# pvjosue/CWFA

Measured on AMD Instinct MI355X. Metric: volumes/sec inverse-pass @512×512×96 fp32; NLL match vs ref (1/2/4/8 GPU), higher is better.
Workload: dtype f32 (storage, accumulation, wavelets, couplings); convolution products on the bf16 matrix cores from an exact three-way bf16 split of both fp32 operands, six products per fp32 product: fp32-equivalent; plain-fp32-MFMA figure: fp32_mfma; 1 GPU; 512x512x96 volume, 4-scale CWFA (CAT blocks, 64 ch) + LRNN inverse, z=0, batch 1/GPU, random-init weights (BASELINE.json configs[2]); precision=split, parallelism=replicated x1 (independent volumes per GPU, no collective)

## Files before the change

cwfa_amd/_lib.py:

```python
import ctypes as C
import os

_HERE = os.path.dirname(os.path.abspath(__file__))
LIB_PATH = os.path.join(_HERE, "libcwfa_hip.so")

CLAMP = {"NONE": 0, "ATAN": 1, "TANH": 2, "SIGMOID": 3}
ACT = {None: 0, "none": 0, "elu": 1, "prelu": 2, "gelu": 3, "relu": 4}
CHAIN_MAX = 8

c_f32p = C.c_void_p
c_i64p = C.c_void_p
c_f64p = C.c_void_p


class AffineStage(C.Structure):
    _fields_ = [("s_raw", c_f32p), ("t", c_f32p), ("s_bs", C.c_int64), ("t_bs", C.c_int64), ("clamp_kind", C.c_int),
                ("clamp", C.c_float), ("pre_scale", C.c_float), ("t_neg_div_sqrt2", C.c_int), ("perm", c_i64p),
                ("perm_axis", C.c_int), ("gin", C.c_int)]


class Chain(C.Structure):
    _fields_ = [("n_stages", C.c_int), ("stage", AffineStage * CHAIN_MAX), ("src_c", C.c_void_p), ("src_h", C.c_void_p)]


# ... 37 lines not shown
    "cwfa_haar2d_inv_f32": (i, [p, p, i, i, i, i, i, f, p]),
    "cwfa_haar3d_fwd_f32": (i, [p, p, i, i, i, i, i, f, i64, p]),
    "cwfa_haar3d_inv_f32": (i, [p, p, i, i, i, i, i, f, i64, p]),
    "cwfa_gather_f32": (i, [p, p, p, i, i, i, i, i, i64, i64, p]),
    "cwfa_affine_f32": (i, [p, p, C.POINTER(AffineStage), i, i, i, i, i, i64, i64, p, p, p]),
    "cwfa_channel_affine_f32": (i, [p, p, p, p, i, p, p, i, i, i64, i64, i64, p]),
    "cwfa_chain_inv_f32": (i, [p, p, p, C.POINTER(Chain), i, i, i, i, i64, i64, i64, p, p]),
    "cwfa_chain_fwd_f32": (i, [p, p, p, C.POINTER(Chain), p, i, i, i, i, i64, i64, i64, p, p, p]),
    "cwfa_conv2d_packed_floats": (i64, [i, i, i]),
    "cwfa_conv2d_pack_f32": (i, [p, p, i, i, i, i, p]),
    "cwfa_conv2d_f32": (i, [p, p, p, i, i, i, i, i, i, i64, i64, C.POINTER(ConvOpts), p]),
    "cwfa_subnet_pack1x1_f32": (i, [p, p, p]),
    "cwfa_subnet_layer_tape_f32": (i, [p, p, p, p, p, p, p, i, i, i, i64, i64, i64, p]),
    "cwfa_subnet_layer_f32": (i, [p, p, p, p, p, p, i, i, i, i64, i64, p]),
    "cwfa_conv3d_1k1_f32": (i, [p, p, p, p, p, p, p, i, i, i, i, i, p]),
    "cwfa_conv3d_1k1_split_f32": (i, [p, p, p, p, p, p, p, i, i, i, i, i, p]),
    "cwfa_channel_stats_f32": (i, [p, p, i, i, i64, i64, p]),
    "cwfa_bn_fold_f32": (i, [p, d, p, p, p, p, f, p, i, p, p, i, p]),
    "cwfa_maxpool_f32": (i, [p, p, p, p, p, i, i, i, i, i, i, p]),
    "cwfa_sample_stats_f32": (i, [p, p, i, i64, p]),
    "cwfa_layernorm_apply_f32": (i, [p, p, p, p, f, p, i, i64, p]),
    "cwfa_attention_combine_f32": (i, [p, p, p, p, p, p, p, p, i, i, i64, p]),
    "cwfa_scale_channels_f32": (i, [p, p, p, i, i, i64, p]),
    "cwfa_axpby_f32": (i, [p, p, f, f, p, i64, p]),
    "cwfa_bn_running_update_f32": (i, [p, C.c_double, f, p, p, p, i, p]),
    "cwfa_bn_finish_f32": (i, [p, d, p, p, p, f, i, p, p, f, p, p, f, f, i, p, p, i, i, p]),
    "cwfa_chain_bwd_f32": (i, [p, p, C.POINTER(Chain), C.POINTER(ChainGrads), p, p, i, i, i, i, i64, i64, i64, f, f, i, p, p]),
    "cwfa_affine_bwd_f32": (i, [p, p, C.POINTER(AffineStage), i, i, i, i, i, i64, i64, p, p, p, p, p]),
    "cwfa_chain_inv_bwd_f32": (i, [p, p, C.POINTER(Chain), C.POINTER(ChainGrads), i, i, i, i, i64, i64, f, i, i, p, p, p, p]),
    "cwfa_conv2d_wgrad_workspace_bytes": (i64, [i, i, i, i, i, i]),
    "cwfa_conv2d_wgrad_f32": (i, [p, p, p, p, p, i, i, i, i, i, i, i64, i64, f, p]),
    "cwfa_elu_bwd_f32": (i, [p, p, p, p, i, i64, i64, i64, i64, i64, p]),
    "cwfa_conv3d_hidden_fwd_f32": (i, [p, p, p, p, i, i, i, i, i, p]),
    "cwfa_conv3d_hidden_bwd_f32": (i, [p, p, p, p, p, p, i, i, i, i, i, p]),
    "cwfa_conv3d_input_bwd_f32": (i, [p, p, p, i, i, i, i, i, p]),
    "cwfa_conv3d_wgrad_workspace_bytes": (i64, [i, i, i, i]),
    "cwfa_conv3d_wgrad_f32": (i, [p, p, p, p, p, i, i, i, i, i, i, i, f, p]),
    "cwfa_prelu_bwd_f32": (i, [p, p, p, p, p, i, i64, i64, i64, i64, p]),
    "cwfa_plane_affine_f32": (i, [p, p, p, i, p, p, i, i, i64, i64, i64, i64, p]),
    "cwfa_bn_bwd_stats_f32": (i, [p, p, p, p, i, i, i64, i64, i64, p]),
    "cwfa_bn_act_bwd_f32": (i, [p, p, p, i, p, p, p, p, p, i, i, i64, i64, i64, i64, p]),
    "cwfa_maxpool2_bwd_f32": (i, [p, p, p, p, i, i, i, i, p]),
    "cwfa_gelu_f32": (i, [p, p, p, i64, i, p]),
    "cwfa_layernorm_bwd_f32": (i, [p, p, p, p, p, p, p, p, p, i, i64, p]),
    "cwfa_attention_bwd_f32": (i, [p, p, p, p, p, p, p, p, p, i, i, i64, p]),
    "cwfa_split_workspace_bytes": (i64, [i, i, i64]),
    "cwfa_split_input_f32": (i, [p, p, i, i, i64, i64, p, p, i64, p, i64, p]),
    "cwfa_conv_split_packed_bytes": (i64, [i, i, i]),
    "cwfa_conv_split_pack_f32": (i, [p, p, i, i, i, i, p]),
    "cwfa_conv_split_f32": (i, [p, p, p, i, i, i, i, i, i, i64, C.POINTER(ConvOpts), p]),
    "cwfa_conv3x3_split_packed_bytes": (i64, [i, i]),
    "cwfa_conv3x3_split_pack_f32": (i, [p, p, i, i, p]),
    "cwfa_conv3x3_split_f32": (i, [p, p, p, i, i, i, i, i, i64, i64, C.POINTER(ConvOpts), p]),
    "cwfa_conv7x7_split_packed_bytes": (i64, [i, i]),
    "cwfa_conv7x7_split_pack_f32": (i, [p, p, i, i, p]),
    "cwfa_conv7x7_split_f32": (i, [p, p, p, i, i, i, i, i, i64, i64, C.POINTER(ConvOpts), p]),
    "cwfa_couple_rows": (i, [i, p]),
    "cwfa_conv3x3_split_couple_f32": (i, [p, p, p, i, i, i, i, i64, C.POINTER(Couple), p]),
    "cwfa_subnet_layer_split_packed_bytes": (i64, []),
    "cwfa_subnet_layer_split_pack_f32": (i, [p, p, p, p]),
    "cwfa_subnet_layer_split_f32": (i, [p, p, p, p, p, i, i, i, i64, i64, i, p]),
    "cwfa_subnet_layer_split_tape_f32": (i, [p, p, p, p, p, p, i, i, i, i64, i64, i64, p]),
    "cwfa_subnet_layer_first_packed_bytes": (i64, []),
    "cwfa_subnet_layer_first_pack_f32": (i, [p, p, p, i, p, p]),
    "cwfa_subnet_layer_first_f32": (i, [p, p, p, p, p, p, i, i, i, i, i64, i64, i64, i, p]),
    "cwfa_extract_views_f32": (i, [p, p, p, i, i, i, i, i, i, f, f, i64, p]),
    "cwfa_eval_splits": (i64, [i, i64]),
    "cwfa_volume_extrema_f32": (i, [p, p, p, p, i, i64, i64, i64, C.POINTER(EvalAffine), p]),
    "cwfa_volume_metrics_f32": (i, [p, p, p, p, i, i64, i64, i64, C.POINTER(EvalAffine), f, f, f, p]),
    "cwfa_mip3_f32": (i, [p, p, p, p, p, p, i, i, i, i, i64, i64, i, C.POINTER(EvalAffine), C.POINTER(EvalPost), p]),
    "cwfa_projection_compose_f32": (i, [p, p, p, p, p, i, i, i, i, i, i, i, p]),
    "cwfa_roi_means_f32": (i, [p, p, p, i, i, i, i, i, i64, p]),
    "cwfa_select_positive_f32": (i, [p, i, i64, i64, i64, p, p, p, p]),
}
del i, i64, f, d, p

_lib = None


class CwfaHipError(RuntimeError):
    pass


def lib():
    global _lib
    if _lib is None:
        if not os.path.exists(LIB_PATH):
            raise CwfaHipError(
                f"{LIB_PATH} not found: build the HIP extension first (python -m cwfa_amd.build, or "
                f"__graft_entry__.build()).  cwfa_amd has no CPU / PyTorch fallback.")
        import torch
        h = C.CDLL(LIB_PATH)
        for name, (res, args) in SIGNATURES.items():
            fn = getattr(h, name)
            fn.restype = res
            fn.argtypes = args
        if h.cwfa_version() < 100:
            raise CwfaHipError("libcwfa_hip.so is older than this Python layer")
        _lib = h
    return _lib


def check(rc, what=""):
    if rc != 0:
        msg = lib().cwfa_last_error()
        raise CwfaHipError(f"{what or 'libcwfa_hip'} failed (code {rc}): {msg.decode() if msg else ''}")
# ... 1 lines not shown
```

cwfa_amd/build.py:

```python
import os
import subprocess
import sys
from concurrent.futures import ThreadPoolExecutor

HERE = os.path.dirname(os.path.abspath(__file__))
CSRC = os.path.join(HERE, "csrc")
INCLUDE = os.path.join(os.path.dirname(HERE), "include")
LIB = os.path.join(HERE, "libcwfa_hip.so")
SOURCES = ["elementwise.hip", "conv2d.hip", "conv_wino.hip", "conv_wino2d.hip", "conv_split_layer.hip", "conv_split3x3.hip", "conv3d.hip", "conv3d_split.hip", "lrnn_ops.hip", "conv_bwd.hip", "eval_ops.hip"]
HIPCC = os.environ.get("HIPCC", "/opt/rocm/bin/hipcc")
FLAGS = ["--offload-arch=gfx950", "-O3", "-fPIC", "-std=c++17", "-ffp-contract=off", "-I", INCLUDE, "-I", CSRC,
         "-Wall", "-Wno-unused-function"]


EXTRA = {"conv3d_split.hip": ["-fno-slp-vectorize"]}


def _newer(src, dst):
    return not os.path.exists(dst) or os.path.getmtime(src) > os.path.getmtime(dst)


def build_all(force=False, verbose=False):
    deps = [os.path.join(CSRC, "common.h"), os.path.join(CSRC, "conv_internal.h"), os.path.join(INCLUDE, "cwfa_hip.h"),
            os.path.abspath(__file__)]
    objs, jobs = [], []
    for s in SOURCES:
        src, obj = os.path.join(CSRC, s), os.path.join(CSRC, s.replace(".hip", ".o"))
        objs.append(obj)
        if force or _newer(src, obj) or any(_newer(d, obj) for d in deps):
            jobs.append([HIPCC, *FLAGS, *EXTRA.get(s, []), "-c", src, "-o", obj])

    def run(cmd):
        if verbose:
            print(" ".join(cmd), flush=True)
        r = subprocess.run(cmd, capture_output=True, text=True)
        if r.returncode != 0:
            raise RuntimeError(f"hipcc failed: {' '.join(cmd)}\n{r.stdout}\n{r.stderr}")
        return r.stderr

    with ThreadPoolExecutor(max_workers=4) as ex:
        for warn in ex.map(run, jobs):
            if verbose and warn.strip():
                print(warn, file=sys.stderr)
    if jobs or force or not os.path.exists(LIB) or any(_newer(o, LIB) for o in objs):
        run([HIPCC, "--offload-arch=gfx950", "-shared", "-fPIC", "-o", LIB, *objs])
    return LIB


if __name__ == "__main__":
    print(build_all(force="--force" in sys.argv, verbose=True))
```

cwfa_amd/csrc/conv2d.hip:

```cpp
#include "conv_internal.h"

#include <string.h>
#include <type_traits>

namespace {

template <int KS_, int CK_, int MT_, int NT_, int WM_, int WN_, int XV_ = 1>
struct Cfg {
    static constexpr int KS = KS_, CK = CK_, MT = MT_, NT = NT_, WM = WM_, WN = WN_;
    static constexpr int XV = XV_;
    static_assert(XV_ == 1 || (XV_ == 4 && KS_ == 1), "vector staging needs halo-free tiles");
    static constexpr int PAD = KS / 2;
    static constexpr int NTHREADS = 64 * WM * WN;
    static constexpr int CT = 32 * MT * WM;
    static constexpr int TR = NT * WN;
    static constexpr int TC = 32;
    static constexpr int XR = TR + KS - 1;
    static constexpr int XC = TC + KS - 1;
    static constexpr int XS = CK * XR * XC;
    static constexpr int XS_PAD = (XS + 3) & ~3;
    static constexpr int WS = KS * KS * CK * CT;
    static constexpr int XPT = (XS / XV + NTHREADS - 1) / NTHREADS;
    static constexpr int WPT = (WS / 4 + NTHREADS - 1) / NTHREADS;
    static constexpr int BUF = XS_PAD + WS;
// ... 503 lines not shown
    p.tiles_y = (p.H + C::TR - 1) / C::TR;
    p.nchunks = (p.Cin + C::CK - 1) / C::CK;
    const int ctiles = (p.Cout + C::CT - 1) / C::CT;
    CWFA_REQUIRE((int64_t)p.tiles_x * p.tiles_y < (1ll << 31) && ctiles <= 65535 && p.B <= 65535, CWFA_E_SHAPE,
                 "cwfa_conv2d_f32: grid too large");
    CWFA_REQUIRE((int64_t)(p.Cin + C::CK) * p.H * p.W * 4 < (1ll << 31), CWFA_E_SHAPE,
                 "cwfa_conv2d_f32: one sample's input must stay below 2 GiB (32-bit buffer offsets)");
    grid = dim3((unsigned)(p.tiles_x * p.tiles_y), ctiles, p.B);
    return CWFA_OK;
}

template <class C, int EPI, bool PRO>
int launch_epi(ConvParams p, hipStream_t stream) {
    dim3 grid;
    int rc = prepare<C>(p, grid);
    if (rc) return rc;
    constexpr int LDS = EPI == EPI_GENERIC && C::LDS_BYTES < C::NTHREADS * 64 ? C::NTHREADS * 64 : C::LDS_BYTES;
    rc = cwfa_max_lds<&conv2d_mfma_kernel<C, EPI, PRO>>(LDS, "cwfa_conv2d_f32");
    if (rc) return rc;
    hipLaunchKernelGGL((conv2d_mfma_kernel<C, EPI, PRO>), grid, dim3(C::NTHREADS), LDS, stream, p);
    CWFA_LAUNCH_CHECK("cwfa_conv2d_f32");
    return CWFA_OK;
}

template <class C, unsigned ALLOWED, bool PRO>
int launch_sel(const ConvParams& p, int epi, hipStream_t st) {
    if (!(ALLOWED & (1u << epi)) && epi != EPI_NONE_BLK8) epi = EPI_GENERIC;
    switch (epi) {
        case EPI_NONE: if constexpr (ALLOWED & (1u << EPI_NONE)) return launch_epi<C, EPI_NONE, PRO>(p, st); break;
        case EPI_ELU: if constexpr (ALLOWED & (1u << EPI_ELU)) return launch_epi<C, EPI_ELU, PRO>(p, st); break;
        case EPI_RES_ELU: if constexpr (ALLOWED & (1u << EPI_RES_ELU)) return launch_epi<C, EPI_RES_ELU, PRO>(p, st); break;
        case EPI_PRELU: if constexpr (ALLOWED & (1u << EPI_PRELU)) return launch_epi<C, EPI_PRELU, PRO>(p, st); break;
        case EPI_RES_PRELU: if constexpr (ALLOWED & (1u << EPI_RES_PRELU)) return launch_epi<C, EPI_RES_PRELU, PRO>(p, st); break;
        case EPI_GELU_RES: if constexpr (ALLOWED & (1u << EPI_GELU_RES)) return launch_epi<C, EPI_GELU_RES, PRO>(p, st); break;
        case EPI_UP: if constexpr (ALLOWED & (1u << EPI_UP)) return launch_epi<C, EPI_UP, PRO>(p, st); break;
        case EPI_NONE_BLK8:
            if constexpr (ALLOWED & (1u << EPI_NONE_BLK8)) return launch_epi<C, EPI_NONE_BLK8, PRO>(p, st);
            cwfa_set_error("cwfa_conv2d_f32: out_blocked8 is built for the 1x1 kernels with more than 32 output channels");
            return CWFA_E_SHAPE;
        default: break;
    }
    return launch_epi<C, EPI_GENERIC, PRO>(p, st);
}

template <class C, unsigned ALLOWED, unsigned ALLOWED_PRO>
int launch(const ConvParams& p, int epi, hipStream_t st) {
    if (p.o.in_scale || p.o.in_add) return launch_sel<C, ALLOWED_PRO, true>(p, epi, st);
    return launch_sel<C, ALLOWED, false>(p, epi, st);
}

}
int g_cwfa_split_xcd_map = 1;
int g_cwfa_split_rows16 = 1;
extern int g_cwfa_mip3_ablate;
namespace {

int fill_params(ConvParams& p, const char* name, const float* x, const float* w_packed, float* y, int B, int Cin, int H,
                int W, int Cout, int64_t x_bs, int64_t y_bs, const cwfa_conv_opts* opts) {
    CWFA_REQUIRE(B >= 0 && Cin > 0 && Cout > 0 && H >= 0 && W >= 0, CWFA_E_INVAL, "%s: bad size", name);
    if (B == 0 || H == 0 || W == 0) return 1;
    CWFA_REQUIRE(x && w_packed && y, CWFA_E_INVAL, "%s: null pointer", name);
    CWFA_REQUIRE((int64_t)Cin * H * W < (1ll << 30) && (int64_t)Cout * H * W * (p.o.upshuffle2 ? 1 : 1) < (1ll << 30), CWFA_E_SHAPE, "%s: C*H*W exceeds the 32-bit byte offsets of a tile (2^30 elements per image)", name);
    CWFA_REQUIRE(cwfa_aligned16(w_packed), CWFA_E_ALIGN, "%s: packed weights must be 16-byte aligned", name);
    p.x = x; p.wp = w_packed; p.y = y;
    p.B = B; p.Cin = Cin; p.H = H; p.W = W; p.Cout = Cout;
    p.x_bs = x_bs; p.y_bs = y_bs;
    p.products = g_cwfa_operand == CwfaOperand::split3 ? 6 : 1;
    if (opts) p.o = *opts;
    CWFA_REQUIRE(!(p.o.in_scale && !p.o.in_shift), CWFA_E_INVAL, "%s: in_scale without in_shift", name);
    CWFA_REQUIRE(p.o.act >= 0 && p.o.act <= CWFA_ACT_RELU && p.o.act2 >= 0 && p.o.act2 <= CWFA_ACT_RELU, CWFA_E_INVAL,
                 "%s: bad activation", name);
    CWFA_REQUIRE(!((p.o.act == CWFA_ACT_PRELU || p.o.act2 == CWFA_ACT_PRELU) && !p.o.prelu_alpha), CWFA_E_INVAL,
                 "%s: PReLU without prelu_alpha", name);
    return CWFA_OK;
}

typedef Cfg<1, 16, 2, 4, 4, 2> CS;
constexpr int CS_XB = 3 * 2 * 8 * 32 * 16, CS_WB = 3 * 2 * 256 * 16, CS_BUFB = CS_XB + CS_WB;

__device__ __forceinline__ void split3(float v, unsigned short (&o)[3]) {
    const __bf16 a1 = (__bf16)v;
    const float r1 = v - (float)a1;
    const __bf16 a2 = (__bf16)r1;
    const float r2 = r1 - (float)a2;
    const __bf16 a3 = (__bf16)r2;
    o[0] = __builtin_bit_cast(unsigned short, a1);
    o[1] = __builtin_bit_cast(unsigned short, a2);
    o[2] = __builtin_bit_cast(unsigned short, a3);
}

__device__ __forceinline__ unsigned short f16_bits(float v) { return __builtin_bit_cast(unsigned short, (_Float16)v); }

template <bool F16 = false>
__global__ __launch_bounds__(256) void split_input_kernel(const float* __restrict__ x, uint4* __restrict__ ws, int Cin, int CG2,
                                                          int64_t HW, int64_t x_bs, const float* __restrict__ sc,
                                                          const float* __restrict__ sh, int64_t aff_bs,
                                                          const float* __restrict__ add, int64_t add_bs) {
    const int64_t px = (int64_t)blockIdx.x * 256 + threadIdx.x;
    if (px >= HW) return;
    const int cg = blockIdx.y, b = blockIdx.z;
    unsigned short pc[3][8];
#pragma unroll
    for (int j = 0; j < 8; ++j) {
        const int c = cg * 8 + j;
        float v = 0.f;
        if (c < Cin) {
// ... 240 lines not shown
    if (rc) return rc < 0 ? rc : CWFA_OK;
    ConvParams& p = sp.c;
    CWFA_REQUIRE(!p.o.in_scale && !p.o.in_add, CWFA_E_INVAL, "cwfa_conv_split_f32: the load-side prologue belongs in cwfa_split_input_f32");
    CWFA_REQUIRE(!p.o.upshuffle2 || (ks == 1 && Cout % 4 == 0), CWFA_E_SHAPE, "cwfa_conv_split_f32: upshuffle2 needs ks=1, Cout=4*Co");
    CWFA_REQUIRE(!p.o.out_stats && !p.o.prelu_per_channel, CWFA_E_INVAL, "cwfa_conv_split_f32: out_stats / prelu_per_channel are features of cwfa_conv3x3_split_f32");
    p.nchunks = (Cin + 15) / 16;
    sp.ws = ws;
    sp.CG2 = 2 * p.nchunks;
    sp.ws_bs = (int64_t)3 * sp.CG2 * H * W * 16;
    CWFA_REQUIRE(sp.ws_bs + (int64_t)4 * H * W * 16 < (1ll << 31) && (int64_t)(p.nchunks * ks * ks + 2) * CS_WB < (1ll << 31), CWFA_E_SHAPE,
                 "cwfa_conv_split_f32: one sample's planes / one cout tile's weights must stay below 2 GiB");
    const int epi = classify_epilogue(p.o);
    hipStream_t st = (hipStream_t)stream;
    switch (epi) {
        case EPI_NONE: return launch_split<EPI_NONE>(sp, st);
        case EPI_UP: return launch_split<EPI_UP>(sp, st);
        default: return launch_split<EPI_GENERIC>(sp, st);
    }
}

int g_cwfa_wino_min_cout = 1;
int g_cwfa_wino_2d = 512;
CwfaOperand g_cwfa_operand = CwfaOperand::split3;

extern "C" int cwfa_set_option(const char* name, int value) {
    CWFA_REQUIRE(name, CWFA_E_INVAL, "cwfa_set_option: null name");
    if (strcmp(name, "winograd_min_cout") == 0) {
        g_cwfa_wino_min_cout = value;
        return CWFA_OK;
    }
    if (strcmp(name, "winograd_2d") == 0) {
        g_cwfa_wino_2d = value;
        return CWFA_OK;
    }
    if (strcmp(name, "wgrad_split") == 0) {
        g_cwfa_wgrad_split = value != 0;
        return CWFA_OK;
    }
    if (strcmp(name, "wgrad_rows") == 0) {
        g_cwfa_wgrad_rows = value;
        return CWFA_OK;
    }
    if (strcmp(name, "split3x3_xcd_map") == 0) {
        g_cwfa_split_xcd_map = value;
        return CWFA_OK;
    }
    if (strcmp(name, "mip3_ablate") == 0) {
        CWFA_REQUIRE(value >= 0 && value <= 7, CWFA_E_INVAL, "cwfa_set_option: mip3_ablate is a mask of bits 0..2");
        g_cwfa_mip3_ablate = value;
        return CWFA_OK;
    }
    if (strcmp(name, "split3x3_rows16") == 0) {
        g_cwfa_split_rows16 = value;
        return CWFA_OK;
    }
    if (strcmp(name, "split_products") == 0) {
        CWFA_REQUIRE(value == 1 || value == 6, CWFA_E_INVAL, "cwfa_set_option: split_products must be 1 or 6");
        CWFA_REQUIRE(value == 1 || g_cwfa_operand != CwfaOperand::fp16, CWFA_E_INVAL,
                     "cwfa_set_option: split_products = 6 needs split_operand = 0 (the three-piece split is a bf16 format)");
        if (value == 6) g_cwfa_operand = CwfaOperand::split3;
        else if (g_cwfa_operand == CwfaOperand::split3) g_cwfa_operand = CwfaOperand::bf16;
        return CWFA_OK;
    }
    if (strcmp(name, "split_operand") == 0) {
        CWFA_REQUIRE(value == 0 || value == 1, CWFA_E_INVAL, "cwfa_set_option: split_operand must be 0 (bf16) or 1 (fp16)");
        CWFA_REQUIRE(value == 0 || g_cwfa_operand != CwfaOperand::split3, CWFA_E_INVAL,
                     "cwfa_set_option: split_operand = 1 (fp16) needs split_products = 1 (fp16 operands take one product)");
        if (value == 1) g_cwfa_operand = CwfaOperand::fp16;
        else if (g_cwfa_operand == CwfaOperand::fp16) g_cwfa_operand = CwfaOperand::bf16;
        return CWFA_OK;
    }
    cwfa_set_error("cwfa_set_option: unknown option '%s'", name);
    return CWFA_E_INVAL;
}

extern "C" int64_t cwfa_conv2d_packed_floats(int Cout, int Cin, int ks) {
    const Sel s = select_cfg(ks, Cout);
    if (s.id < 0 || Cout <= 0 || Cin <= 0) return -1;
    if (cwfa_wino_selected(ks, Cout)) return cwfa_wino_packed_floats(Cout, Cin);
    const int64_t ctiles = (Cout + s.CT - 1) / s.CT, nchunks = (Cin + s.CK - 1) / s.CK;
    return ctiles * nchunks * ks * ks * s.CK * s.CT;
}

extern "C" int cwfa_conv2d_pack_f32(const float* w, float* packed, int Cout, int Cin, int ks, int transposed, void* stream) {
    CWFA_REQUIRE(w && packed, CWFA_E_INVAL, "cwfa_conv2d_pack_f32: null pointer");
    CWFA_REQUIRE(!transposed || (ks == 1 && Cout % 4 == 0), CWFA_E_SHAPE,
                 "cwfa_conv2d_pack_f32: transposed source needs ks=1 (2x2 stride-2 deconv as 1x1) and Cout = 4*Co");
    const int64_t total = cwfa_conv2d_packed_floats(Cout, Cin, ks);
    CWFA_REQUIRE(total > 0, CWFA_E_SHAPE, "cwfa_conv2d_pack_f32: unsupported filter %dx%d, Cout=%d, Cin=%d", ks, ks, Cout, Cin);
    if (cwfa_wino_selected(ks, Cout)) return cwfa_wino_pack(w, packed, Cout, Cin, (hipStream_t)stream);
    const Sel s = select_cfg(ks, Cout);
    const int nchunks = (Cin + s.CK - 1) / s.CK;
    hipLaunchKernelGGL(pack_kernel, dim3((unsigned)((total + 255) / 256)), dim3(256), 0, (hipStream_t)stream, w, packed, Cout,
                       Cin, ks, s.CT, s.CK, nchunks, total, transposed);
    CWFA_LAUNCH_CHECK("cwfa_conv2d_pack_f32");
    return CWFA_OK;
}

extern "C" int cwfa_conv2d_f32(const float* x, const float* w_packed, float* y, int B, int Cin, int H, int W, int Cout, int ks,
                               int64_t x_bs, int64_t y_bs, const cwfa_conv_opts* opts, void* stream) {
    CWFA_REQUIRE(!(opts && opts->in_blocked8), CWFA_E_INVAL, "cwfa_conv2d_f32: in_blocked8 is a cwfa_conv3x3_split_f32 feature");
    CWFA_REQUIRE(!(opts && opts->in_cat) || (ks == 1 && Cout <= 64 && !opts->in_scale && !opts->in_add && opts->in_cat_from % 16 == 0 &&
                                             opts->in_cat_from > 0 && opts->in_cat_from < Cin && opts->in_cat_c1 > 0 &&
                                             opts->in_cat_c1 <= opts->in_cat_from),
                 CWFA_E_INVAL, "cwfa_conv2d_f32: in_cat needs a 1x1 bank with <= 64 outputs packed with in_cat_from (a multiple of 16) "
                               "columns for the first source, and no load-side affine / add");
// ... 83 lines not shown
```

cwfa_amd/ops.py:

```python
import ctypes as C

import torch

from . import _lib
from ._lib import AffineStage, Chain, ConvOpts, check

__all__ = ["haar1d", "haar2d", "gather", "affine", "channel_affine", "chain_inv", "chain_fwd", "pack_conv_weight",
           "conv2d", "conv2d_wgrad", "elu_bwd", "set_precision", "gelu_add", "gelu_bwd", "layernorm_bwd", "attention_bwd", "plane_affine", "bn_bwd_stats", "bn_act_bwd", "maxpool2_bwd", "chain_bwd", "chain_inv_bwd", "prelu_bwd", "conv3d_1k1_backward", "pack_1x1_panel", "pack_split_layer_weight", "subnet_layer", "conv3d_1k1", "channel_stats", "bn_fold", "bn_running_update", "maxpool", "sample_stats", "layernorm_apply",
           "attention_combine", "scale_channels", "axpby", "stage"]


def _stream():
    return C.c_void_p(torch.cuda.current_stream().cuda_stream)


def _p(t):
    return None if t is None else C.c_void_p(t.data_ptr())


def _dev(t, name="tensor"):
    if not torch.is_tensor(t):
        raise TypeError(f"{name}: expected a torch.Tensor, got {type(t)}")
    if not t.is_cuda:
        raise RuntimeError(f"{name}: cwfa_amd runs on MI355X only -- got a {t.device} tensor (no CPU fallback exists)")
# ... 430 lines not shown
            raise ValueError("conv2d: in_add shape mismatch")
        o.in_add, o.in_add_bs = in_add.data_ptr(), abs_
        keep.append(in_add)
    o.upshuffle2 = int(up)
    if in_blocked:
        if not (pc.split and pc.ks == 3):
            raise ValueError("conv2d: channel-blocked input is read by the split-bf16 3x3 kernel only")
        o.in_blocked8 = 1
    if out_blocked:
        ok3 = (pc.split and pc.ks == 3 and pc.cout % 8 == 0 and residual is None and act2 is None and act in (None, "prelu")
               and not split3x3_narrow(pc.cout) and not (in_add is not None and act is None))
        ok1 = not pc.split and pc.ks == 1 and pc.cout >= 33 and pc.cout % 8 == 0 and not up
        if not (ok3 or ok1):
            raise ValueError("conv2d: channel-blocked output is written by the split-bf16 3x3 kernel (bias / PReLU) and by the "
                             "direct 1x1 kernel with 40..64 output channels only")
        o.out_blocked8 = 1
    if out_stats is not None:
        if not conv_writes_stats(pc, act, residual, act2, out_blocked, in_add is not None):
            raise ValueError("conv2d: out_stats needs the split-bf16 3x3 kernel with an NCHW output and a bias / PReLU epilogue")
        if out_stats.dtype != torch.float64 or out_stats.numel() != 2 * pc.cout or not out_stats.is_cuda:
            raise ValueError("conv2d: out_stats must be a float64 [2*Cout] tensor on the HIP device")
        o.out_stats = out_stats.data_ptr()
    rec = conv_event_sink
    if rec is not None:
        key = (pc.ks, Cin, pc.cout, H, W, B, "%s|%s|%s|%s|%s" % ("pro" if (in_scale is not None or in_add is not None) else "",
                                                                 act or "", "res" if residual is not None else "", act2 or "",
                                                                 ("up" if up else "") + ("+split" if pc.split else "")),
               in_add is not None)
        if rec.want(key):
            e0, e1 = torch.cuda.Event(enable_timing=True), torch.cuda.Event(enable_timing=True)
            e0.record()
    if pc.split and pc.ks == 7:
        if act or act2 or residual is not None or in_scale is not None or in_add is not None:
            raise ValueError("conv2d: the split-bf16 7x7 kernel has a bias-only epilogue and no load-side prologue")
        check(L.cwfa_conv7x7_split_f32(_p(x), _p(pc.packed), _p(out), B, Cin, H, W, pc.cout, xbs, ybs, C.byref(o), _stream()),
              "conv7x7_split")
    elif pc.split and pc.ks == 3:
        if split3x3_narrow(pc.cout) and (in_scale is not None or in_add is not None):
            if (H * W) % 4 == 0:
                x = plane_affine(x, in_scale, in_shift, add=in_add)
            else:
                if in_scale is not None:
                    if in_scale.numel() == Cin:
                        x = channel_affine(x, in_scale.reshape(-1), in_shift.reshape(-1))
                    else:
                        x = torch.cat([channel_affine(x[i:i + 1], in_scale.reshape(B, Cin)[i].contiguous(), in_shift.reshape(B, Cin)[i].contiguous())
                                       for i in range(B)], 0)
                if in_add is not None:
                    x = axpby(x.contiguous(), 1.0, in_add, 1.0)
            x, xbs = planes(x, "x")
            o.in_scale = o.in_shift = o.in_add = None
        check(L.cwfa_conv3x3_split_f32(_p(x), _p(pc.packed), _p(out), B, Cin, H, W, pc.cout, xbs, ybs, C.byref(o),
                                       _stream()), "conv3x3_split")
    elif pc.split:
        ws = torch.empty(L.cwfa_split_workspace_bytes(B, Cin, H * W), dtype=torch.uint8, device=x.device)
        per_sample = in_scale is not None and in_scale.numel() == B * Cin and B > 1
        check(L.cwfa_split_input_f32(_p(x), _p(ws), B, Cin, H * W, xbs, _p(in_scale), _p(in_shift), Cin if per_sample else 0,
                                     _p(in_add), in_add.stride(0) if in_add is not None else 0, _stream()), "split_input")
        o.in_scale = o.in_shift = o.in_add = None
        check(L.cwfa_conv_split_f32(_p(ws), _p(pc.packed), _p(out), B, Cin, H, W, pc.cout, pc.ks, ybs, C.byref(o), _stream()),
              "conv_split")
    else:
        check(L.cwfa_conv2d_f32(_p(x), _p(pc.packed), _p(out), B, Cin, H, W, pc.cout, pc.ks, xbs, ybs, C.byref(o),
                                _stream()), "conv2d")
    if rec is not None and rec.want(key):
        e1.record()
        rec.add(key, e0, e1)
    return out


def pack_couple_weight(w, bias):
    L = _lib.lib()
    w = _dev(w, "weight").detach()
    n2, cin, ks, kw = w.shape
    if ks != 3 or kw != 3 or n2 % 2 or n2 // 2 > 64:
        raise ValueError(f"pack_couple_weight: a [2n,Cin,3,3] bank with n <= 64 is needed, got {tuple(w.shape)}")
    n = n2 // 2
    total = L.cwfa_couple_rows(n, None)
    rows_c = (C.c_int * total)()
    L.cwfa_couple_rows(n, rows_c)
    rows = torch.tensor(list(rows_c), dtype=torch.int64, device=w.device)
    live = (rows >= 0)
    wr = torch.zeros((total, cin, 3, 3), dtype=torch.float32, device=w.device)
    wr[live] = w[rows[live]]
    br = torch.zeros(total, dtype=torch.float32, device=w.device)
    if bias is not None:
        br[live] = _dev(bias, "bias").detach()[rows[live]]
    packed = torch.empty(L.cwfa_conv3x3_split_packed_bytes(total, cin), dtype=torch.uint8, device=w.device)
    check(L.cwfa_conv3x3_split_pack_f32(_p(wr), _p(packed), total, cin, _stream()), "conv3x3_split_pack (coupling bank)")
    pc = PackedConv(packed, n2, cin, 3, False, w._version, w.data_ptr(), split=True)
    pc.version1, pc.src_ptr1 = (bias._version, bias.data_ptr()) if bias is not None else (None, None)
    return pc, br


def conv3x3_couple(u, pc_bias, x, out, clamp_kind, clamp, pre_scale, rev, logdet=None, in_blocked=False):
    L = _lib.lib()
    pc, br = pc_bias
    u, ubs = planes(u, "u")
    B, Cin, H, W = u.shape
    n = pc.cout // 2
    if Cin != pc.cin:
        raise ValueError(f"conv3x3_couple: input has {Cin} channels, filter bank expects {pc.cin}")
    x2, xbs = planes(x, "x")
    o2, obs = planes(out, "out")
    if tuple(x.shape) != (B, n, H, W) or tuple(out.shape) != (B, n, H, W) or o2.data_ptr() != out.data_ptr():
        raise ValueError("conv3x3_couple: x / out must be [B,n,H,W] views with contiguous planes")
# ... 547 lines not shown
    check(L.cwfa_attention_combine_f32(_p(mean), _p(_dev(w1).contiguous()), _p(_dev(b1)), _p(_dev(w2).contiguous()),
                                       _p(_dev(b2)), _p(m), _p(x), _p(out), B, Cc, HW, _stream()), "attention_combine")
    return out


def scale_channels(x, scale_bc):
    L = _lib.lib()
    x = _dev(x, "x").contiguous()
    B, Cc = x.shape[:2]
    if scale_bc.numel() != B * Cc:
        raise ValueError(f"scale_channels: the table must hold B*C = {B * Cc} factors")
    out = torch.empty_like(x)
    check(L.cwfa_scale_channels_f32(_p(x), _p(_dev(scale_bc).contiguous()), _p(out), B, Cc, x[0, 0].numel(), _stream()),
          "scale_channels")
    return out


def axpby(x, a, z=None, b=0.0):
    L = _lib.lib()
    x = _dev(x, "x").contiguous()
    z = None if z is None else _dev(z).contiguous()
    if z is not None and z.numel() != x.numel():
        raise ValueError("axpby: x and z differ in size")
    out = torch.empty_like(x)
    check(L.cwfa_axpby_f32(_p(x), _p(z), float(a), float(b), _p(out), x.numel(), _stream()), "axpby")
    return out


def extract_views(image, coords_yx, subimage_shape, mean=0.0, std=1.0):
    L = _lib.lib()
    image = _dev(image, "image")
    if image.dim() != 4 or image.shape[1] != 1:
        raise ValueError(f"extract_views: image must be [B,1,H,W], got {tuple(image.shape)}")
    if image.dtype != torch.float32:
        raise TypeError("extract_views: fp32 images only")
    image = image if image[0].is_contiguous() else image.contiguous()
    B, _, Hs, Ws = image.shape
    co = torch.as_tensor(coords_yx, dtype=torch.int32).reshape(-1, 2)
    sh, sw = int(subimage_shape[0]), int(subimage_shape[1])
    ys, xs = co[:, 0], co[:, 1]
    if len(co) and (bool(((torch.minimum(ys + sh // 2, torch.tensor(Hs)) - torch.clamp(ys - sh // 2, min=0)) <= 0).any()) or
                    bool(((torch.minimum(xs + sw // 2, torch.tensor(Ws)) - torch.clamp(xs - sw // 2, min=0)) <= 0).any())):
        raise ValueError("extract_views: a lenslet window lies outside the image")
    cod = co.contiguous().to(image.device)
    out = torch.empty((B, len(co), sh, sw), dtype=torch.float32, device=image.device)
    check(L.cwfa_extract_views_f32(_p(image), _p(cod), _p(out), B, Hs, Ws, len(co), sh, sw, float(mean), float(std),
                                   image.stride(0), _stream()), "extract_views")
    return out


_split_bf16 = 0
_precision = "fp32"
_pack_epoch = 0


def single_product():
    return _precision in ("bf16", "fp16")


def pack_epoch():
    return _pack_epoch


def invalidate_packs():
    global _pack_epoch
    _pack_epoch += 1


WINOGRAD_2D_DEFAULT = 512


def set_option(name, value):
    global _split_bf16, _pack_epoch
    _pack_epoch += 1
    if name == "split_bf16":
        _split_bf16 = int(value)
        return
    check(_lib.lib().cwfa_set_option(name.encode(), int(value)), "set_option")


PRECISIONS = ("fp32", "split_bf16", "bf16", "fp16")


def set_precision(mode):
    if mode not in PRECISIONS:
        raise ValueError(f"set_precision: unknown mode {mode!r}")
    global _precision
    _precision = mode
    set_option("split_operand", 0)
    set_option("split_products", 1 if single_product() else 6)
    if mode == "fp16":
        set_option("split_operand", 1)
    set_option("split_bf16", 0 if mode == "fp32" else 2)
    set_option("wgrad_split", 0 if mode == "fp32" else 1)


def copy_channels(src, dst):
    L = _lib.lib()
    s_, sbs = planes(src, "src")
    d_, dbs = planes(dst, "dst")
    if d_.data_ptr() != dst.data_ptr() or tuple(src.shape) != tuple(dst.shape):
        raise ValueError("copy_channels: dst must be a [B,c,H,W] view with contiguous planes of src's shape")
    B, Cc, H, W = s_.shape
    check(L.cwfa_channel_affine_f32(_p(s_), _p(dst), None, None, 0, None, None, B, Cc, H * W, sbs, dbs, _stream()), "copy_channels")
    return dst


def concat_channels(parts):
    L = _lib.lib()
    parts = [planes(t, "part") for t in parts]
    B, _, H, W = parts[0][0].shape
    Ct = sum(t.shape[1] for t, _ in parts)
    out = torch.empty((B, Ct, H, W), dtype=torch.float32, device=parts[0][0].device)
    c0 = 0
    for t, bs in parts:
        if t.shape[0] != B or t.shape[2:] != (H, W):
            raise ValueError("concat_channels: shape mismatch")
        check(L.cwfa_channel_affine_f32(_p(t), C.c_void_p(out.data_ptr() + 4 * c0 * H * W), None, None, 0, None, None, B,
                                        t.shape[1], H * W, bs, Ct * H * W, _stream()), "concat_channels")
        c0 += t.shape[1]
    return out


def eval_affine(step, mean, std):
    a = _lib.EvalAffine()
    a.enabled, a.scale = 1, 2.0 ** -int(step)
    a.std = float(torch.as_tensor(std, dtype=torch.float32).reshape(()).cpu())
# ... 89 lines not shown
```

include/cwfa_hip.h:

```cpp
#ifndef CWFA_HIP_H
#define CWFA_HIP_H

#include <stdint.h>

#ifdef __cplusplus
extern "C" {
#endif

#define CWFA_VERSION 100

enum {
    CWFA_OK = 0,
    CWFA_E_INVAL = -1,
    CWFA_E_SHAPE = -2,
    CWFA_E_ALIGN = -3,
    CWFA_E_HIP = -4
};

enum { CWFA_CLAMP_NONE = 0, CWFA_CLAMP_ATAN = 1, CWFA_CLAMP_TANH = 2, CWFA_CLAMP_SIGMOID = 3 };

enum { CWFA_ACT_NONE = 0, CWFA_ACT_ELU = 1, CWFA_ACT_PRELU = 2, CWFA_ACT_GELU = 3, CWFA_ACT_RELU = 4 };

int cwfa_version(void);
const char* cwfa_last_error(void);
// ... 80 lines not shown
    int64_t in_cat_bs;
    int in_cat_from, in_cat_c1;
    double* out_stats;
    int prelu_per_channel;
} cwfa_conv_opts;

int cwfa_conv2d_f32(const float* x, const float* w_packed, float* y, int B, int Cin, int H, int W, int Cout, int ks,
                    int64_t x_bs, int64_t y_bs, const cwfa_conv_opts* opts, void* stream);

int cwfa_subnet_pack1x1_f32(const float* w, float* panel, void* stream);
int cwfa_subnet_layer_f32(const float* x, const float* w3_packed, const float* b3, const float* w1_panel, const float* b1,
                          float* y, int B, int H, int W, int64_t x_bs, int64_t y_bs, void* stream);
int cwfa_subnet_layer_tape_f32(const float* x, const float* w3_packed, const float* b3, const float* w1_panel, const float* b1,
                               float* y, float* hidden, int B, int H, int W, int64_t x_bs, int64_t y_bs, int64_t hidden_bs,
                               void* stream);

int cwfa_conv3d_1k1_f32(const float* x, const float* w1, const float* b1, const float* alpha, const float* w2,
                        const float* b2, float* y, int B, int D, int H, int W, int K, void* stream);
int cwfa_conv3d_1k1_split_f32(const float* x, const float* w1, const float* b1, const float* alpha, const float* w2,
                              const float* b2, float* y, int B, int D, int H, int W, int K, void* stream);


int cwfa_channel_stats_f32(const float* x, double* stats, int B, int C, int64_t HW, int64_t x_bs, void* stream);
int cwfa_bn_fold_f32(const double* stats, double count, const float* running_mean, const float* running_var,
                     const float* weight, const float* bias, float eps, const float* mask_bc, int B, float* scale,
                     float* shift, int C, void* stream);
int cwfa_bn_finish_f32(double* stats, double count, float* running_mean, float* running_var, long long* num_batches_tracked,
                       float momentum, int update_running, const float* weight, const float* bias, float eps, const float* mask_bc,
                       const float* mask_u, float drop_p, float keep_scale, int B, float* scale, float* shift, int C, int zero_stats,
                       void* stream);
int cwfa_bn_running_update_f32(const double* stats, double count, float momentum, float* running_mean, float* running_var,
                               long long* num_batches_tracked, int C, void* stream);
int cwfa_maxpool_f32(const float* x, float* y, float* full, const float* scale, const float* shift, int B, int C,
                     int H, int W, int Ho, int Wo, void* stream);
int cwfa_sample_stats_f32(const float* x, double* stats, int B, int64_t CHW, void* stream);
int cwfa_layernorm_apply_f32(const float* x, const double* stats, const float* w, const float* b, float eps,
                             float* y, int B, int64_t CHW, void* stream);
int cwfa_attention_combine_f32(const float* mean, const float* w1, const float* b1, const float* w2, const float* b2,
                               const float* m, const float* x, float* out, int B, int C, int64_t HW, void* stream);
int cwfa_scale_channels_f32(const float* x, const float* scale_bc, float* y, int B, int C, int64_t HW, void* stream);
int cwfa_axpby_f32(const float* x, const float* z, float a, float b, float* y, int64_t n, void* stream);

int64_t cwfa_split_workspace_bytes(int B, int Cin, int64_t HW);
int cwfa_split_input_f32(const float* x, void* ws, int B, int Cin, int64_t HW, int64_t x_bs, const float* in_scale,
                         const float* in_shift, int64_t in_affine_bs, const float* in_add, int64_t in_add_bs, void* stream);
int64_t cwfa_conv_split_packed_bytes(int Cout, int Cin, int ks);
int cwfa_conv_split_pack_f32(const float* w, void* packed, int Cout, int Cin, int ks, int transposed, void* stream);
int64_t cwfa_conv3x3_split_packed_bytes(int Cout, int Cin);
int cwfa_conv3x3_split_pack_f32(const float* w, void* packed, int Cout, int Cin, void* stream);
int cwfa_conv3x3_split_f32(const float* x, const void* w_packed, float* y, int B, int Cin, int H, int W, int Cout,
                           int64_t x_bs, int64_t y_bs, const cwfa_conv_opts* opts, void* stream);
int cwfa_conv_split_f32(const void* ws, const void* w_packed, float* y, int B, int Cin, int H, int W, int Cout, int ks, int64_t y_bs,
                           const cwfa_conv_opts* opts, void* stream);
int64_t cwfa_conv7x7_split_packed_bytes(int Cout, int Cin);
int cwfa_conv7x7_split_pack_f32(const float* w, void* packed, int Cout, int Cin, void* stream);
int cwfa_conv7x7_split_f32(const float* x, const void* w_packed, float* y, int B, int Cin, int H, int W, int Cout,
                           int64_t x_bs, int64_t y_bs, const cwfa_conv_opts* opts, void* stream);

typedef struct {
    const float* x;
    float* y;
    int64_t x_bs, y_bs;
    int n;
    int clamp_kind;
    float clamp, pre_scale;
    int rev;
    double* logdet;
    int in_blocked8;
} cwfa_couple;
int cwfa_couple_rows(int n, int* rows);
int cwfa_conv3x3_split_couple_f32(const float* x, const void* w_packed, const float* bias_rows, int B, int Cin, int H, int W,
                                  int64_t x_bs, const cwfa_couple* cp, void* stream);

int64_t cwfa_subnet_layer_split_packed_bytes(void);
int cwfa_subnet_layer_split_pack_f32(const float* w3, const float* w1, void* packed, void* stream);
int cwfa_subnet_layer_split_f32(const float* x, const void* packed, const float* b3, const float* b1, float* y, int B, int H,
                                int W, int64_t x_bs, int64_t y_bs, int layout, void* stream);
int64_t cwfa_subnet_layer_first_packed_bytes(void);
int cwfa_subnet_layer_first_pack_f32(const float* w3c, const float* w1, const float* w0c, int short_form, void* packed, void* stream);
int cwfa_subnet_layer_first_f32(const float* u, const float* x, const void* packed, const float* b3, const float* b1, float* y, int B,
                                int u_ch, int H, int W, int64_t u_bs, int64_t x_bs, int64_t y_bs, int layout, void* stream);
int cwfa_subnet_layer_split_tape_f32(const float* x, const void* packed, const float* b3, const float* b1, float* y, float* hid, int B,
                                     int H, int W, int64_t x_bs, int64_t y_bs, int64_t hid_bs, void* stream);

int cwfa_extract_views_f32(const float* image, const int* coords_yx, float* views, int B, int Hs, int Ws, int nviews, int sh,
                           int sw, float mean, float stdv, int64_t image_bs, void* stream);


typedef struct {
    float* ds[CWFA_CHAIN_MAX];
    float* dt[CWFA_CHAIN_MAX];
    int64_t ds_bs[CWFA_CHAIN_MAX], dt_bs[CWFA_CHAIN_MAX];
} cwfa_chain_grads;

int cwfa_chain_bwd_f32(const float* z, const float* gz, const cwfa_chain* ch, const cwfa_chain_grads* grads,
                       const int64_t* final_perm, float* gv0, int B, int C, int H, int W, int64_t z_bs, int64_t gz_bs,
                       int64_t gv0_bs, float gscale, float ldscale, int accumulate, const float* gld, void* stream);

int cwfa_chain_inv_bwd_f32(const float* xhat, const float* gt, const cwfa_chain* ch, const cwfa_chain_grads* grads, int B, int C,
                           int H, int W, int64_t xhat_bs, int64_t gt_bs, float gscale, int loss_kind, int accumulate,
                           double* loss_sum, float* gz_out, float* glow_out, void* stream);

int cwfa_affine_bwd_f32(const float* x, const float* g, const cwfa_affine_stage* st, int rev, int B, int C, int H, int W,
                        int64_t x_bs, int64_t g_bs, const float* gld, float* gx, float* gs_raw, float* gt_raw, void* stream);

int64_t cwfa_conv2d_wgrad_workspace_bytes(int B, int Cin, int H, int W, int Cout, int ks);
// ... 65 lines not shown
```

Before: 52.65 volumes/s.

## Add fused split-on-load upsampling conv kernel for transposed 2x2 banks

Adds a dedicated kernel for the upshuffle (transposed 2x2) split-precision convolution. It loads fp32 input, applies the affine prologue and does the three-way bf16 split in registers before writing to LDS. Weight DMA and the next tile's input loads are overlapped with the MFMA loop, and the output is pixel-shuffled directly in the epilogue. This removes the separate split-workspace pass and its global-memory round trip. The cost is a large-LDS, single-block-per-CU kernel, and the new path has its own correctness surface.

```diff
diff --git a/cwfa_amd/_lib.py b/cwfa_amd/_lib.py
--- a/cwfa_amd/_lib.py
+++ b/cwfa_amd/_lib.py
@@ -113,6 +113,7 @@
     "cwfa_conv3x3_split_packed_bytes": (i64, [i, i]),
     "cwfa_conv3x3_split_pack_f32": (i, [p, p, i, i, p]),
     "cwfa_conv3x3_split_f32": (i, [p, p, p, i, i, i, i, i, i64, i64, C.POINTER(ConvOpts), p]),
+    "cwfa_conv_up_split_f32": (i, [p, p, p, i, i, i, i, i, i64, i64, C.POINTER(ConvOpts), p]),
     "cwfa_conv7x7_split_packed_bytes": (i64, [i, i]),
     "cwfa_conv7x7_split_pack_f32": (i, [p, p, i, i, p]),
     "cwfa_conv7x7_split_f32": (i, [p, p, p, i, i, i, i, i, i64, i64, C.POINTER(ConvOpts), p]),
diff --git a/cwfa_amd/build.py b/cwfa_amd/build.py
--- a/cwfa_amd/build.py
+++ b/cwfa_amd/build.py
@@ -7,7 +7,7 @@
 CSRC = os.path.join(HERE, "csrc")
 INCLUDE = os.path.join(os.path.dirname(HERE), "include")
 LIB = os.path.join(HERE, "libcwfa_hip.so")
-SOURCES = ["elementwise.hip", "conv2d.hip", "conv_wino.hip", "conv_wino2d.hip", "conv_split_layer.hip", "conv_split3x3.hip", "conv3d.hip", "conv3d_split.hip", "lrnn_ops.hip", "conv_bwd.hip", "eval_ops.hip"]
+SOURCES = ["elementwise.hip", "conv2d.hip", "conv_wino.hip", "conv_wino2d.hip", "conv_split_layer.hip", "conv_split3x3.hip", "conv_split_up.hip", "conv3d.hip", "conv3d_split.hip", "lrnn_ops.hip", "conv_bwd.hip", "eval_ops.hip"]
 HIPCC = os.environ.get("HIPCC", "/opt/rocm/bin/hipcc")
 FLAGS = ["--offload-arch=gfx950", "-O3", "-fPIC", "-std=c++17", "-ffp-contract=off", "-I", INCLUDE, "-I", CSRC,
          "-Wall", "-Wno-unused-function"]
diff --git a/cwfa_amd/csrc/conv2d.hip b/cwfa_amd/csrc/conv2d.hip
--- a/cwfa_amd/csrc/conv2d.hip
+++ b/cwfa_amd/csrc/conv2d.hip
@@ -579,6 +579,7 @@
 }
 int g_cwfa_split_xcd_map = 1;
 int g_cwfa_split_rows16 = 1;
+int g_cwfa_split_up_onload = 1;
 extern int g_cwfa_mip3_ablate;
 namespace {
 
@@ -925,6 +926,10 @@
     }
     if (strcmp(name, "split3x3_rows16") == 0) {
         g_cwfa_split_rows16 = value;
+        return CWFA_OK;
+    }
+    if (strcmp(name, "split_up_onload") == 0) {
+        g_cwfa_split_up_onload = value != 0;
         return CWFA_OK;
     }
     if (strcmp(name, "split_products") == 0) {
diff --git a/cwfa_amd/csrc/conv_split_up.hip b/cwfa_amd/csrc/conv_split_up.hip
--- /dev/null
+++ b/cwfa_amd/csrc/conv_split_up.hip
@@ -0,0 +1,270 @@
+#include "conv_internal.h"
+
+extern int g_cwfa_split_xcd_map;
+extern int g_cwfa_split_up_onload;
+
+namespace {
+
+constexpr int TR = 8, TC = 32, NPX = TR * TC;
+constexpr int MPW = 4, CT = 256;
+constexpr int KGB = NPX * 16 + 64;
+constexpr int XPB = 4 * KGB;
+constexpr int XB = 3 * XPB;
+constexpr int CHB = 3 * 2 * CT * 16;
+constexpr int WSL = 2 * CHB;
+constexpr int LDS_BYTES = XB + 2 * WSL;
+static_assert(LDS_BYTES <= 160 * 1024, "LDS budget");
+
+struct UParams {
+    const float* x;
+    const void* wp;
+    float* y;
+    const float *bias, *in_scale, *in_shift;
+    int64_t in_affine_bs, x_bs, y_bs;
+    int B, Cin, H, W, Cout, nchunks, nsteps, tiles_x, ntiles, ctiles, xcd_map;
+};
+
+template <bool SIX, bool F16>
+__global__ __launch_bounds__(512, 1) void conv_up_split_kernel(UParams p) {
+    extern __shared__ __attribute__((aligned(16))) char lds[];
+    const int tid = threadIdx.x, lane = tid & 63, c16 = lane & 15, g = lane >> 4;
+    const int wave = __builtin_amdgcn_readfirstlane(tid >> 6);
+    const int wm = wave & 3, wn = wave >> 2;
+    const int HW = p.H * p.W, plane = HW * 4;
+    constexpr unsigned OOB = 0x80000000u;
+    constexpr int NQ = SIX ? 3 : 1;
+    constexpr int OFF_W = XB;
+    const int b = blockIdx.z;
+    int sp, ct;
+    if (p.xcd_map && (p.ntiles & 7) == 0) {
+        const int xcd = blockIdx.x & 7, slot = blockIdx.x >> 3;
+        sp = xcd * (p.ntiles >> 3) + slot / p.ctiles;
+        ct = slot % p.ctiles;
+    } else {
+        sp = blockIdx.x / p.ctiles;
+        ct = blockIdx.x % p.ctiles;
+    }
+    const int row0 = (sp / p.tiles_x) * TR, col0 = (sp % p.tiles_x) * TC;
+
+    const int spx = tid & (NPX - 1), kgw = (wave >> 2) * 2;
+    const int sgr = row0 + (spx >> 5), sgc = col0 + (spx & 31);
+    const unsigned fo = (sgr < p.H && sgc < p.W) ? (unsigned)((sgr * p.W + sgc) * 4) : OOB;
+    const auto rx = CWFA_RSRC(p.x + (int64_t)b * p.x_bs, p.Cin * plane);
+    const bool has_aff = p.in_scale != nullptr;
+    typedef const float __attribute__((address_space(4))) cfloat;
+    cfloat* sc = has_aff ? (cfloat*)(p.in_scale + (int64_t)b * p.in_affine_bs) : nullptr;
+    cfloat* sh = has_aff ? (cfloat*)(p.in_shift + (int64_t)b * p.in_affine_bs) : nullptr;
+    char* const sdst = lds + kgw * KGB + spx * 16;
+
+    float xs[2][8], scv[2][8], shv[2][8];
+    bf16x8 pcs[2][3];
+    auto load_tile = [&](int step) {
+#pragma unroll
+        for (int k = 0; k < 2; ++k)
+#pragma unroll
+            for (int j = 0; j < 8; ++j)
+                xs[k][j] = __builtin_bit_cast(float, __builtin_amdgcn_raw_buffer_load_b32(rx, fo, (step * 32 + (kgw + k) * 8 + j) * plane, 0));
+        if (has_aff) {
+#pragma unroll
+            for (int k = 0; k < 2; ++k) {
+                const int ch0 = step * 32 + (kgw + k) * 8;
+                if (ch0 + 8 <= p.Cin) {
+#pragma unroll
+                    for (int j = 0; j < 8; ++j) {
+                        scv[k][j] = sc[ch0 + j];
+                        shv[k][j] = sh[ch0 + j];
+                    }
+                } else {
+#pragma unroll
+                    for (int j = 0; j < 8; ++j) {
+                        const bool in = ch0 + j < p.Cin;
+                        const int ch = in ? ch0 + j : p.Cin - 1;
+                        scv[k][j] = in ? sc[ch] : 0.f;
+                        shv[k][j] = in ? sh[ch] : 0.f;
+                    }
+                }
+            }
+        }
+    };
+    auto split_tile = [&]() {
+#pragma unroll
+        for (int k = 0; k < 2; ++k) {
+#pragma unroll
+            for (int j = 0; j < 8; ++j) {
+                float v = xs[k][j];
+                if (has_aff) v = v * scv[k][j] + shv[k][j];
+                __bf16 a1, a2 = (__bf16)0.f, a3 = (__bf16)0.f;
+                cwfa_split3<SIX, F16>(v, a1, a2, a3);
+                pcs[k][0][j] = a1; pcs[k][1][j] = a2; pcs[k][2][j] = a3;
+            }
+        }
+    };
+    auto store_tile = [&]() {
+#pragma unroll
+        for (int k = 0; k < 2; ++k)
+#pragma unroll
+            for (int q = 0; q < NQ; ++q) *reinterpret_cast<bf16x8*>(sdst + k * KGB + q * XPB) = pcs[k][q];
+    };
+
+    constexpr int NPC = SIX ? WSL / 1024 : 16;
+    const char* wbase = reinterpret_cast<const char*>(p.wp) + (int64_t)ct * p.nchunks * CHB;
+    const auto rw = CWFA_RSRC(wbase, p.nchunks * CHB);
+    auto dma_w = [&](int slice, int slot) {
+        cwfa_static_for<NPC / 8>([&](auto ic_) {
+            constexpr int i = decltype(ic_)::value;
+            const int piece = i * 8 + wave;
+            const int off = SIX ? piece * 1024 : (piece >> 3) * CHB + (piece & 7) * 1024;
+            char* dst = lds + OFF_W + slot * WSL + off;
+            __builtin_amdgcn_raw_ptr_buffer_load_lds(rw, (lds_ptr)dst, 16, (unsigned)(lane * 16), slice * WSL + off, 0, 0);
+        });
+    };
+
+    const int alane = OFF_W + (g >> 1) * CHB + (g & 1) * (CT * 16) + (wm * MPW * 16 + c16) * 16;
+    const int blane = g * KGB + (wn * 4 * TC + c16) * 16;
+    constexpr int NT = 8, MH = 2;
+
+    f32x4 acc[MPW][NT];
+#pragma unroll
+    for (int mt = 0; mt < MPW; ++mt)
+#pragma unroll
+        for (int nt = 0; nt < NT; ++nt) acc[mt][nt] = f32x4{0.f, 0.f, 0.f, 0.f};
+    bf16x8 A[MH][3], Bq[2][3];
+
+    auto read_a = [&](int abase, int m0) {
+#pragma unroll
+        for (int mt = 0; mt < MH; ++mt)
+#pragma unroll
+            for (int q = 0; q < NQ; ++q) A[mt][q] = *reinterpret_cast<const bf16x8*>(lds + abase + q * (2 * CT * 16) + (m0 + mt) * 256);
+    };
+    auto read_b = [&](int set, int nt) {
+#pragma unroll
+        for (int q = 0; q < NQ; ++q)
+            Bq[set][q] = *reinterpret_cast<const bf16x8*>(lds + blane + q * XPB + ((nt >> 1) * TC + 16 * (nt & 1)) * 16);
+    };
+    auto mfma6 = [&](f32x4& c, const bf16x8 (&a)[3], const bf16x8 (&bb)[3]) {
+        if constexpr (SIX) {
+            CWFA_MFMA(a[2], bb[0], c);
+            CWFA_MFMA(a[1], bb[1], c);
+            CWFA_MFMA(a[0], bb[2], c);
+            CWFA_MFMA(a[1], bb[0], c);
+            CWFA_MFMA(a[0], bb[1], c);
+        }
+        CWFA_MFMA_OP(F16, a[0], bb[0], c);
+    };
+
+    load_tile(0);
+    dma_w(0, 0);
+    split_tile();
+    store_tile();
+    asm volatile("s_waitcnt vmcnt(0)\n\ts_waitcnt lgkmcnt(0)" ::: "memory");
+    __builtin_amdgcn_s_barrier();
+
+    int sl = 0;
+    for (int step = 0; step < p.nsteps; ++step) {
+        const int abase = alane + sl * WSL;
+        read_a(abase, 0);
+        read_b(0, 0);
+        CWFA_FENCE();
+#pragma unroll
+        for (int m0 = 0; m0 < MPW; m0 += MH) {
+            if (m0 > 0) {
+                read_a(abase, m0);
+                read_b(0, 0);
+                CWFA_FENCE();
+            }
+#pragma unroll
+            for (int nt = 0; nt < NT; ++nt) {
+                if (nt + 1 < NT) read_b((nt + 1) & 1, nt + 1);
+                CWFA_FENCE();
+#pragma unroll
+                for (int mt = 0; mt < MH; ++mt) {
+                    mfma6(acc[m0 + mt][nt], A[mt], Bq[nt & 1]);
+                    CWFA_FENCE();
+                }
+                if (m0 == 0 && nt == 0) {
+                    load_tile(step + 1);
+                    CWFA_FENCE();
+                }
+                if (m0 == 0 && nt == 1) {
+                    dma_w(step + 1, sl ^ 1);
+                    CWFA_FENCE();
+                }
+            }
+        }
+        asm volatile("s_waitcnt vmcnt(0)" ::: "memory");
+        split_tile();
+        CWFA_FENCE();
+        asm volatile("s_waitcnt lgkmcnt(0)" ::: "memory");
+        __builtin_amdgcn_s_barrier();
+        store_tile();
+        asm volatile("s_waitcnt lgkmcnt(0)" ::: "memory");
+        __builtin_amdgcn_s_barrier();
+        sl ^= 1;
+    }
+
+    const int Co = p.Cout >> 2, plane2 = 4 * plane, W2 = 2 * p.W;
+    const auto ry = CWFA_RSRC(p.y + (int64_t)b * p.y_bs, Co * plane2);
+    const auto rb = CWFA_RSRC(p.bias ? p.bias : p.y, p.bias ? Co * 4 : 0);
+    const int cwave = ct * (CT / 4) + wm * MPW * 4;
+    const unsigned glane = (unsigned)g * (unsigned)plane2;
+    typedef unsigned u32x2 __attribute__((ext_vector_type(2)));
+#pragma unroll
+    for (int mt = 0; mt < MPW; ++mt) {
+        const float bias = __builtin_bit_cast(float, __builtin_amdgcn_raw_buffer_load_b32(rb, (unsigned)(4 * g), (cwave + mt * 4) * 4, 0));
+#pragma unroll
+        for (int nt = 0; nt < NT; ++nt) {
+            const int row = row0 + wn * 4 + (nt >> 1), col = col0 + 16 * (nt & 1) + c16;
+            const unsigned po = (row < p.H && col < p.W) ? (unsigned)((2 * row * W2 + 2 * col) * 4) + glane : OOB;
+            const unsigned po1 = po != OOB ? po + (unsigned)(W2 * 4) : OOB;
+            u32x2 lo, hi;
+            lo[0] = __builtin_bit_cast(unsigned, acc[mt][nt][0] + bias);
+            lo[1] = __builtin_bit_cast(unsigned, acc[mt][nt][1] + bias);
+            hi[0] = __builtin_bit_cast(unsigned, acc[mt][nt][2] + bias);
+            hi[1] = __builtin_bit_cast(unsigned, acc[mt][nt][3] + bias);
+            __builtin_amdgcn_raw_buffer_store_b64(lo, ry, po, (cwave + mt * 4) * plane2, 0);
+            __builtin_amdgcn_raw_buffer_store_b64(hi, ry, po1, (cwave + mt * 4) * plane2, 0);
+            CWFA_FENCE();
+        }
+    }
+}
+
+}
+
+extern "C" int cwfa_conv_up_split_f32(const float* x, const void* w_packed, float* y, int B, int Cin, int H, int W, int Cout,
+                                      int64_t x_bs, int64_t y_bs, const cwfa_conv_opts* opts, void* stream) {
+    CWFA_REQUIRE(B >= 0 && Cin > 0 && Cout > 0 && H >= 0 && W >= 0, CWFA_E_INVAL, "cwfa_conv_up_split_f32: bad size");
+    CWFA_REQUIRE(g_cwfa_split_up_onload, CWFA_E_INVAL, "cwfa_conv_up_split_f32: switched off (option split_up_onload)");
+    CWFA_REQUIRE(Cout % 4 == 0, CWFA_E_SHAPE, "cwfa_conv_up_split_f32: Cout = 4 * Co packed rows (got %d)", Cout);
+    if (B == 0 || H == 0 || W == 0) return CWFA_OK;
+    CWFA_REQUIRE(x && w_packed && y, CWFA_E_INVAL, "cwfa_conv_up_split_f32: null pointer");
+    CWFA_REQUIRE(cwfa_aligned16(w_packed), CWFA_E_ALIGN, "cwfa_conv_up_split_f32: packed weights must be 16-byte aligned");
+    cwfa_conv_opts o{};
+    if (opts) o = *opts;
+    CWFA_REQUIRE(o.upshuffle2 && !o.in_add && !o.in_cat && !o.in_blocked8 && !o.out_blocked8 && !o.residual && !o.out_stats &&
+                     o.act == CWFA_ACT_NONE && o.act2 == CWFA_ACT_NONE,
+                 CWFA_E_INVAL, "cwfa_conv_up_split_f32: transposed banks with a bias-only epilogue and an affine-only prologue");
+    CWFA_REQUIRE(!o.in_scale == !o.in_shift, CWFA_E_INVAL, "cwfa_conv_up_split_f32: in_scale and in_shift go together");
+    UParams p{};
+    p.x = x; p.wp = w_packed; p.y = y;
+    p.bias = o.bias; p.in_scale = o.in_scale; p.in_shift = o.in_shift; p.in_affine_bs = o.in_affine_bs;
+    p.B = B; p.Cin = Cin; p.H = H; p.W = W; p.Cout = Cout; p.x_bs = x_bs; p.y_bs = y_bs;
+    p.nchunks = (Cin + 15) / 16;
+    p.nsteps = (Cin + 31) / 32;
+    p.tiles_x = (W + TC - 1) / TC;
+    p.ntiles = p.tiles_x * ((H + TR - 1) / TR);
+    p.ctiles = (Cout + CT - 1) / CT;
+    p.xcd_map = g_cwfa_split_xcd_map;
+    CWFA_REQUIRE((int64_t)(Cin + 64) * H * W * 4 < (1ll << 31) && (int64_t)(Cout / 4 + CT / 4) * H * W * 16 < (1ll << 31) &&
+                     (int64_t)(p.nsteps + 2) * WSL < (1ll << 31), CWFA_E_SHAPE,
+                 "cwfa_conv_up_split_f32: one sample's input / output / one cout tile's weights must stay below 2 GiB");
+    CWFA_REQUIRE((int64_t)p.tiles_x * ((H + TR - 1) / TR) * p.ctiles < (1ll << 31) && B <= 65535, CWFA_E_SHAPE,
+                 "cwfa_conv_up_split_f32: grid too large");
+    return cwfa_with_operand([&](auto six, auto f16) -> int {
+        constexpr auto kern = &conv_up_split_kernel<six, f16>;
+        const int rc = cwfa_max_lds<kern>(LDS_BYTES, "cwfa_conv_up_split_f32");
+        if (rc) return rc;
+        hipLaunchKernelGGL(kern, dim3((unsigned)(p.ntiles * p.ctiles), 1, B), dim3(512), LDS_BYTES, (hipStream_t)stream, p);
+        CWFA_LAUNCH_CHECK("cwfa_conv_up_split_f32");
+        return CWFA_OK;
+    });
+}
diff --git a/cwfa_amd/ops.py b/cwfa_amd/ops.py
--- a/cwfa_amd/ops.py
+++ b/cwfa_amd/ops.py
@@ -506,6 +506,9 @@
             o.in_scale = o.in_shift = o.in_add = None
         check(L.cwfa_conv3x3_split_f32(_p(x), _p(pc.packed), _p(out), B, Cin, H, W, pc.cout, xbs, ybs, C.byref(o),
                                        _stream()), "conv3x3_split")
+    elif pc.split and up and _split_up_onload and in_add is None and act is None and act2 is None and residual is None:
+        check(L.cwfa_conv_up_split_f32(_p(x), _p(pc.packed), _p(out), B, Cin, H, W, pc.cout, xbs, ybs, C.byref(o), _stream()),
+              "conv_up_split")
     elif pc.split:
         ws = torch.empty(L.cwfa_split_workspace_bytes(B, Cin, H * W), dtype=torch.uint8, device=x.device)
         per_sample = in_scale is not None and in_scale.numel() == B * Cin and B > 1
@@ -1159,6 +1162,7 @@
 _split_bf16 = 0
 _precision = "fp32"
 _pack_epoch = 0
+_split_up_onload = True
 
 
 def single_product():
@@ -1178,8 +1182,10 @@
 
 
 def set_option(name, value):
-    global _split_bf16, _pack_epoch
+    global _split_bf16, _pack_epoch, _split_up_onload
     _pack_epoch += 1
+    if name == "split_up_onload":
+        _split_up_onload = bool(value)
     if name == "split_bf16":
         _split_bf16 = int(value)
         return
diff --git a/include/cwfa_hip.h b/include/cwfa_hip.h
--- a/include/cwfa_hip.h
+++ b/include/cwfa_hip.h
@@ -156,6 +156,8 @@
                            int64_t x_bs, int64_t y_bs, const cwfa_conv_opts* opts, void* stream);
 int cwfa_conv_split_f32(const void* ws, const void* w_packed, float* y, int B, int Cin, int H, int W, int Cout, int ks, int64_t y_bs,
                            const cwfa_conv_opts* opts, void* stream);
+int cwfa_conv_up_split_f32(const float* x, const void* w_packed, float* y, int B, int Cin, int H, int W, int Cout,
+                           int64_t x_bs, int64_t y_bs, const cwfa_conv_opts* opts, void* stream);
 int64_t cwfa_conv7x7_split_packed_bytes(int Cout, int Cin);
 int cwfa_conv7x7_split_pack_f32(const float* w, void* packed, int Cout, int Cin, void* stream);
 int cwfa_conv7x7_split_f32(const float* x, const void* w_packed, float* y, int B, int Cin, int H, int W, int Cout,
```

Result: no change. 52.90 volumes/s, median of 6 (+0.5%).
